# google-research/hyperbo

Hardware: AMD Instinct MI355X
Metric: GP NLL+grad evals/sec at N=8192 D=16 fp64 (higher is better)
Workload: dtype f64

## Files before the change

hyperbo_amd/csrc/chol.hip:

```cpp
#include "hbo_internal.h"
#include <type_traits>
#include <limits.h>
#include <string.h>

namespace {

#include "panel_dev.h"
#ifdef HBO_POTF2_TIMING
__device__ unsigned long long hbo_dbg_stamps[64];
__device__ unsigned long long hbo_dbg_wall[3 * 256];
__device__ unsigned long long hbo_dbg_trsm[3 * 128];
__device__ int hbo_dbg_trsm_panel = 36;
#define STAMP(i) do { if (threadIdx.x == 0) hbo_dbg_stamps[i] = __builtin_readcyclecounter(); } while (0)
#else
#define STAMP(i) do {} while (0)
#endif
#ifndef HBO_POTF2_WAVES
#define HBO_POTF2_WAVES 8
#endif
constexpr int POTF2_WAVES = HBO_POTF2_WAVES;
constexpr int POTF2_THREADS = 64 * POTF2_WAVES;
template <typename T>
__device__ __forceinline__ void potf2_body(const TaskDesc& t, int p, int* info_slot, unsigned char* smem) {
  typedef typename Mma<T>::acc_t acc_t;
  T* sT = reinterpret_cast<T*>(smem);
  T* sM = sT + 36 * TILE_ELEMS;
  T* sDinv = sM + TILE_ELEMS;
  const int64_t ld = t.ld;
  T* Ab = static_cast<T*>(t.A) + (int64_t)p * NB * ld + (int64_t)p * NB;
  T* Wb = static_cast<T*>(t.W) + (int64_t)p * NB * ld + (int64_t)p * NB;
  const int tid = threadIdx.x, lane = tid & 63, wave = tid >> 6;
  const int l15 = lane & 15, lq = lane >> 4;
  const int ei = (tid & 255) >> 4, ej = tid & 15;
  STAMP(0);
#ifdef HBO_POTF2_TIMING
  if (tid == 0 && blockIdx.x == 0 && p < 256) {
    hbo_dbg_wall[3 * p] = wall_clock64();
    hbo_dbg_wall[3 * p + 2] = ((unsigned long long)__builtin_amdgcn_s_getreg((20 << 0) | (0 << 6) | (31 << 11)) << 32) |
                              (unsigned)__builtin_amdgcn_s_getreg((4 << 0) | (0 << 6) | (31 << 11));
  }
#endif

  auto factor_leaf = [&](int jb, const acc_t* from_regs = nullptr) {
    T* dt = sT + tri_index(jb, jb) * TILE_ELEMS;
    acc_t acc;
    if (from_regs) acc = *from_regs;
    else {
#pragma unroll
      for (int r = 0; r < 4; ++r) acc[r] = dt[Mma<T>::crow(lane, r) * TS + l15];
    }
    const int bad = leaf_cholesky4<T>(acc, dt, sM, sDinv + jb * 16, Wb + (int64_t)(jb * 16) * ld + jb * 16, ld, lane);
    if (bad >= 0 && lane == 0) atomicMin(info_slot, p * NB + jb * 16 + bad + 1);
  };
  auto solve_tile = [&](int jb, int R) {
    T* xt = sT + tri_index(R, jb) * TILE_ELEMS;
    acc_t acc = {0, 0, 0, 0};
#pragma unroll
    for (int kk = 0; kk < 4; ++kk) acc = Mma<T>::mma(xt[l15 * TS + kk * 4 + lq], sM[l15 * TS + kk * 4 + lq], acc);
#pragma unroll
    for (int r = 0; r < 4; ++r) xt[Mma<T>::crow(lane, r) * TS + l15] = acc[r];
  };
  auto update_tile = [&](int jb, int I, int J) {
    T* ct = sT + tri_index(I, J) * TILE_ELEMS;
    const T* at = sT + tri_index(I, jb) * TILE_ELEMS;
    const T* bt = sT + tri_index(J, jb) * TILE_ELEMS;
    acc_t acc;
#pragma unroll
    for (int r = 0; r < 4; ++r) acc[r] = ct[Mma<T>::crow(lane, r) * TS + l15];
#pragma unroll
    for (int kk = 0; kk < 4; ++kk) acc = Mma<T>::mma(-at[l15 * TS + kk * 4 + lq], bt[l15 * TS + kk * 4 + lq], acc);
#pragma unroll
    for (int r = 0; r < 4; ++r) ct[Mma<T>::crow(lane, r) * TS + l15] = acc[r];
  };

  auto update_tile2 = [&](int jb, int I0, int J0, int I1, int J1) {
    T* c0 = sT + tri_index(I0, J0) * TILE_ELEMS;
    T* c1 = sT + tri_index(I1, J1) * TILE_ELEMS;
    const T* a0 = sT + tri_index(I0, jb) * TILE_ELEMS;
    const T* b0 = sT + tri_index(J0, jb) * TILE_ELEMS;
    const T* a1 = sT + tri_index(I1, jb) * TILE_ELEMS;
    const T* b1 = sT + tri_index(J1, jb) * TILE_ELEMS;
    acc_t x0, x1;
    T fa0[4], fb0[4], fa1[4], fb1[4];
#pragma unroll
    for (int r = 0; r < 4; ++r) { x0[r] = c0[Mma<T>::crow(lane, r) * TS + l15]; x1[r] = c1[Mma<T>::crow(lane, r) * TS + l15]; }
#pragma unroll
    for (int kk = 0; kk < 4; ++kk) {
      fa0[kk] = -a0[l15 * TS + kk * 4 + lq]; fb0[kk] = b0[l15 * TS + kk * 4 + lq];
      fa1[kk] = -a1[l15 * TS + kk * 4 + lq]; fb1[kk] = b1[l15 * TS + kk * 4 + lq];
    }
#pragma unroll
    for (int kk = 0; kk < 4; ++kk) { x0 = Mma<T>::mma(fa0[kk], fb0[kk], x0); x1 = Mma<T>::mma(fa1[kk], fb1[kk], x1); }
#pragma unroll
    for (int r = 0; r < 4; ++r) { c0[Mma<T>::crow(lane, r) * TS + l15] = x0[r]; c1[Mma<T>::crow(lane, r) * TS + l15] = x1[r]; }
  };

  int nleaf = 8;
  {
    const int64_t rows = (int64_t)t.n - (int64_t)p * NB;
    if (rows < NB) nleaf = rows <= 0 ? 0 : (int)((rows + 15) / 16);
    for (int jb = nleaf + wave; jb < 8; jb += POTF2_WAVES)
#pragma unroll
      for (int r = 0; r < 4; ++r) {
        const int row = Mma<T>::crow(lane, r);
        gst(Wb + (int64_t)(jb * 16 + row) * ld + jb * 16 + l15, row == l15 ? (T)1 : (T)0);
      }
    if (tid < NB && tid >= nleaf * 16) sDinv[tid] = (T)1;
  }
  const bool lead_tile0 = nleaf > 0;
  acc_t tile0 = {0, 0, 0, 0};
  if (wave == 0 && lead_tile0) {
#pragma unroll
    for (int r = 0; r < 4; ++r) {
      const int row = Mma<T>::crow(lane, r);
      const int rr = row > l15 ? row : l15, cc = row > l15 ? l15 : row;
      tile0[r] = gld(Ab + (int64_t)rr * ld + cc);
    }
  }
  constexpr int NSH = POTF2_THREADS / 256;
  const int sh = __builtin_amdgcn_readfirstlane(tid >> 8);
  T vload[36 / NSH];
  auto load_issue = [&](auto share) {
    constexpr int SH = decltype(share)::value;
    int tile = 0;
#pragma unroll
    for (int I = 0; I < 8; ++I)
#pragma unroll
      for (int J = 0; J <= I; ++J, ++tile) {
        if (tile % NSH != SH) continue;
        if (tile == 0 && lead_tile0) { vload[0] = (T)0; continue; }
        int r = ei, c = ej;
        if (I == J && ej > ei) { r = ej; c = ei; }
        vload[tile / NSH] = gld(Ab + (int64_t)(I * 16 + r) * ld + J * 16 + c);
      }
  };
  auto load_commit = [&](auto share) {
    constexpr int SH = decltype(share)::value;
#pragma unroll
    for (int k = 0; k < 36 / NSH; ++k)
      if (!(k == 0 && SH == 0 && lead_tile0)) sT[(k * NSH + SH) * TILE_ELEMS + ei * TS + ej] = vload[k];
  };
  static_assert(NSH == 1 || NSH == 2, "one or two 256-thread groups");
  if (NSH == 1 || sh == 0) load_issue(std::integral_constant<int, 0>());
  else load_issue(std::integral_constant<int, NSH - 1>());
  if (wave == 0 && lead_tile0) factor_leaf(0, &tile0);
  if (NSH == 1 || sh == 0) load_commit(std::integral_constant<int, 0>());
  else load_commit(std::integral_constant<int, NSH - 1>());
  STAMP(1);
  __syncthreads();
  STAMP(2);
  for (int jb = 0; jb < nleaf; ++jb) {
    for (int R = jb + 1 + wave; R < nleaf; R += POTF2_WAVES) solve_tile(jb, R);
    __syncthreads();
    STAMP(3 + 3 * jb);
    if (jb == nleaf - 1) break;
    {
      const int m = nleaf - 1 - jb;
      const int ntiles = m * (m + 1) / 2;
      constexpr int NH = POTF2_WAVES == 8 ? 6 : POTF2_WAVES - 1;
      const int hw = POTF2_WAVES == 8 ? (wave < 4 ? wave : wave - 1) : wave;
      const int n0 = (ntiles - 1 > 4 * NH + 1) ? (ntiles - 1 - (4 * NH + 1)) / POTF2_WAVES : 0;
      const int nshared = ntiles - n0;
      auto tile_of = [&](int tix, int& I, int& J) {
        int ii = 0;
        while ((ii + 1) * (ii + 2) / 2 <= tix) ++ii;
        I = jb + 1 + ii; J = jb + 1 + tix - ii * (ii + 1) / 2;
      };
      if (wave == 0) {
        update_tile(jb, jb + 1, jb + 1);
        factor_leaf(jb + 1);
        STAMP(4 + 3 * jb);
        for (int tix = nshared; tix < ntiles; ++tix) { int I, J; tile_of(tix, I, J); update_tile(jb, I, J); }
      } else if (!(POTF2_WAVES == 8 && wave == 4)) {
        int tix = hw;
        for (; tix + NH < nshared; tix += 2 * NH) {
          int I0, J0, I1, J1;
          tile_of(tix, I0, J0); tile_of(tix + NH, I1, J1);
          update_tile2(jb, I0, J0, I1, J1);
        }
        if (tix < nshared) { int I, J; tile_of(tix, I, J); update_tile(jb, I, J); }
      }
    }
    __syncthreads();
    STAMP(5 + 3 * jb);
  }
  STAMP(30);

  auto store_share = [&](auto share) {
    constexpr int SH = decltype(share)::value;
    int tile = 0;
#pragma unroll
    for (int I = 0; I < 8; ++I)
#pragma unroll
      for (int J = 0; J <= I; ++J, ++tile) {
        if (tile % NSH != SH) continue;
        T v = sT[tile * TILE_ELEMS + ei * TS + ej];
        if (I == J && ej > ei) v = (T)0;
        gst(Ab + (int64_t)(I * 16 + ei) * ld + J * 16 + ej, v);
      }
  };
  if (NSH == 1 || sh == 0) store_share(std::integral_constant<int, 0>());
  else store_share(std::integral_constant<int, NSH - 1>());
  STAMP(31);
  STAMP(32);
#ifdef HBO_POTF2_TIMING
  if (tid == 0 && blockIdx.x == 0 && p < 256) hbo_dbg_wall[3 * p + 1] = wall_clock64();
#endif
}
template <typename T>
__global__ __launch_bounds__(POTF2_THREADS) void potf2_kernel(const TaskDesc* tasks, int p, int* info, int* yield_flag, unsigned long long* tl) {
  extern __shared__ __attribute__((aligned(16))) unsigned char smem[];
  __builtin_amdgcn_s_setprio(3);
  const TaskDesc& t = tasks[blockIdx.x];
  if (p >= t.nblk) return;
  tl_begin(tl);
  int tok = 0;
  if (yield_flag && threadIdx.x == 0) tok = yield_enter(yield_flag);
  potf2_body<T>(t, p, info + blockIdx.x, smem);
  if (yield_flag) {
    __syncthreads();
    if (threadIdx.x == 0) yield_leave(yield_flag, tok);
  }
  tl_end(tl);
}

template <typename T>
constexpr int trsm_tile() { return sizeof(T) == 8 ? 256 : TILE_ELEMS; }
template <typename T>
__device__ __forceinline__ int trsm_at(int r, int c) { return sizeof(T) == 8 ? r * 16 + (c ^ ((r >> 1) << 1)) : r * TS + c; }
template <typename T>
constexpr int trsm_lds_bytes() { return (28 + 8 + 4) * trsm_tile<T>() * (int)sizeof(T); }
__device__ __forceinline__ int strict_index(int I, int J) { return I * (I - 1) / 2 + J; }

template <typename T, bool IDENT>
__device__ __forceinline__ void trsm_body(const TaskDesc& t, int p, int64_t row0, unsigned char* smem, bool stage) {
  typedef typename Mma<T>::acc_t acc_t;
  constexpr int TE = trsm_tile<T>();
  T* sLt = reinterpret_cast<T*>(smem);
  T* sWi = sLt + 28 * TE;
  T* sSc = sWi + 8 * TE;
  const int64_t ld = t.ld;
  const int tid = threadIdx.x, lane = tid & 63, wave = tid >> 6;
  const int l15 = lane & 15, lq = lane >> 4;
  const T* Lb = static_cast<const T*>(t.A) + (int64_t)p * NB * ld + (int64_t)p * NB;
  const T* Wb = static_cast<const T*>(t.W) + (int64_t)p * NB * ld + (int64_t)p * NB;

  const int64_t wrow0 = row0 + wave * 16;
  const int rg = IDENT ? (int)((wrow0 - (int64_t)p * NB) >> 4) : 0;
  T* Ap = IDENT ? nullptr : static_cast<T*>(t.A) + wrow0 * ld + (int64_t)p * NB;
  T* Wout = IDENT ? static_cast<T*>(t.W) + (int64_t)p * NB * ld + (int64_t)p * NB : nullptr;

  acc_t areg[8];
#pragma unroll
  for (int jb = 0; jb < 8; ++jb)
#pragma unroll
    for (int r = 0; r < 4; ++r) {
      const int row = Mma<T>::crow(lane, r);
      if (IDENT) areg[jb][r] = (rg == jb && row == l15) ? (T)1 : (T)0;
      else areg[jb][r] = gld(Ap + (int64_t)row * ld + jb * 16 + l15);
    }
  if (stage) {
    const int i = tid >> 4, j = tid & 15;
    int tile = 0;
#pragma unroll
    for (int I = 1; I < 8; ++I)
#pragma unroll
      for (int J = 0; J < I; ++J, ++tile)
        sLt[tile * TE + trsm_at<T>(i, j)] = gld(Lb + (int64_t)(I * 16 + i) * ld + J * 16 + j);
#pragma unroll
    for (int b = 0; b < 8; ++b)
      sWi[b * TE + trsm_at<T>(i, j)] = gld(Wb + (int64_t)(b * 16 + i) * ld + b * 16 + j);
  }
  if (stage) __syncthreads();

  T* sc = sSc + wave * TE;
  T xneg[8][4];
#pragma unroll
  for (int jb = 0; jb < 8; ++jb) {
    acc_t acc = areg[jb];
    acc_t acc2 = (acc_t){0, 0, 0, 0};
#pragma unroll
    for (int kb = 0; kb < 8; ++kb) {
      if (kb < jb) {
        const T* lt = sLt + strict_index(jb, kb) * TE;
#pragma unroll
        for (int kk = 0; kk < 4; ++kk) {
          const T bfrag = lt[trsm_at<T>(l15, kk * 4 + lq)];
          if (kb & 1) acc2 = Mma<T>::mma(xneg[kb][kk], bfrag, acc2);
          else acc = Mma<T>::mma(xneg[kb][kk], bfrag, acc);
        }
      }
    }
#pragma unroll
    for (int r = 0; r < 4; ++r) acc[r] += acc2[r];
    __builtin_amdgcn_wave_barrier();
#pragma unroll
    for (int r = 0; r < 4; ++r) sc[trsm_at<T>(Mma<T>::crow(lane, r), l15)] = acc[r];
    __builtin_amdgcn_wave_barrier();
    T ta[4];
#pragma unroll
    for (int kk = 0; kk < 4; ++kk) ta[kk] = sc[trsm_at<T>(l15, kk * 4 + lq)];
    acc_t x = (acc_t){0, 0, 0, 0};
    const T* wt = sWi + jb * TE;
#pragma unroll
    for (int kk = 0; kk < 4; ++kk) {
      const T bfrag = wt[trsm_at<T>(l15, kk * 4 + lq)];
      x = Mma<T>::mma(ta[kk], bfrag, x);
    }
#pragma unroll
    for (int r = 0; r < 4; ++r) {
      const int row = Mma<T>::crow(lane, r);
      if (IDENT) {
        if (rg != jb) gst(Wout + (int64_t)(jb * 16 + l15) * ld + rg * 16 + row, x[r]);
      } else {
        gst(Ap + (int64_t)row * ld + jb * 16 + l15, x[r]);
      }
    }
    if (jb < 7) {
      __builtin_amdgcn_wave_barrier();
#pragma unroll
      for (int r = 0; r < 4; ++r) sc[trsm_at<T>(Mma<T>::crow(lane, r), l15)] = x[r];
      __builtin_amdgcn_wave_barrier();
#pragma unroll
      for (int kk = 0; kk < 4; ++kk) xneg[jb][kk] = -sc[trsm_at<T>(l15, kk * 4 + lq)];
    }
  }
}
template <typename T, bool IDENT>
__global__ __launch_bounds__(256) void trsm_kernel(const TaskDesc* tasks, int p_arg, int* yield_tab, unsigned long long* tl) {
  extern __shared__ __attribute__((aligned(16))) unsigned char smem[];
  __builtin_amdgcn_s_setprio(3);
  const TaskDesc& t = tasks[blockIdx.z];
  const int p = IDENT ? p_arg + (int)blockIdx.y : p_arg;
  if (p >= t.nblk) return;
#ifdef HBO_POTF2_TIMING
  const bool dbg = !IDENT && p == hbo_dbg_trsm_panel && blockIdx.x < 128 && threadIdx.x == 0;
  if (dbg) {
    hbo_dbg_trsm[3 * blockIdx.x] = wall_clock64();
    hbo_dbg_trsm[3 * blockIdx.x + 2] = ((unsigned long long)__builtin_amdgcn_s_getreg((20 << 0) | (0 << 6) | (31 << 11)) << 32) |
                                       (unsigned)__builtin_amdgcn_s_getreg((4 << 0) | (0 << 6) | (31 << 11));
  }
#endif
  int64_t row0;
  if (IDENT) {
    row0 = (int64_t)p * NB + (int64_t)blockIdx.x * 64;
  } else {
    const int64_t first = (int64_t)(p + 1) * NB;
    const int64_t nrows = (int64_t)(t.nblk + 1) * NB - first;
    const int64_t bx = ((int64_t)blockIdx.x + 3 * (int64_t)blockIdx.z) % gridDim.x;
    if (bx * 64 >= nrows) return;
    row0 = first + bx * 64;
  }
  int tok = 0;
  tl_begin(tl);
  if (yield_tab && threadIdx.x == 0) tok = yield_enter(yield_tab);
  trsm_body<T, IDENT>(t, p, row0, smem, true);
  if (yield_tab) {
    __syncthreads();
    if (threadIdx.x == 0) yield_leave(yield_tab, tok);
  }
  tl_end(tl);
#ifdef HBO_POTF2_TIMING
  if (dbg) hbo_dbg_trsm[3 * blockIdx.x + 1] = wall_clock64();
#endif
}

template <typename T>
void set_attrs() {
  static unsigned long long seen = 0;
  if (!hbo_first_use_on_device(seen)) return;
  hipFuncSetAttribute(reinterpret_cast<const void*>(&potf2_kernel<T>),
                      hipFuncAttributeMaxDynamicSharedMemorySize, potf2_lds_bytes<T>());
  hipFuncSetAttribute(reinterpret_cast<const void*>(&trsm_kernel<T, false>),
                      hipFuncAttributeMaxDynamicSharedMemorySize, trsm_lds_bytes<T>());
  hipFuncSetAttribute(reinterpret_cast<const void*>(&trsm_kernel<T, true>),
                      hipFuncAttributeMaxDynamicSharedMemorySize, trsm_lds_bytes<T>());
}

template <typename T>
void potf2_t(const TaskDesc* tasks, int ntasks, int p, int* info, hipStream_t st, int* yield_flag, unsigned long long* tl) {
  set_attrs<T>();
  hipLaunchKernelGGL((potf2_kernel<T>), dim3(ntasks), dim3(POTF2_THREADS), potf2_lds_bytes<T>(), st, tasks, p, info,
                     yield_flag, tl);
}
template <typename T>
void trsm_t(const TaskDesc* tasks, int ntasks, int p, int max_nblk, hipStream_t st, int* yield_tab, unsigned long long* tl) {
  set_attrs<T>();
  const int nrows = (max_nblk + 1 - (p + 1)) * NB;
  if (nrows <= 0) return;
  hipLaunchKernelGGL((trsm_kernel<T, false>), dim3(nrows / 64, 1, ntasks), dim3(256), trsm_lds_bytes<T>(), st,
                     tasks, p, yield_tab, tl);
}
template <typename T>
void trtri_diag_t(const TaskDesc* tasks, int ntasks, int p_lo, int p_hi, hipStream_t st) {
  set_attrs<T>();
  if (p_hi <= p_lo) return;
  hipLaunchKernelGGL((trsm_kernel<T, true>), dim3(2, p_hi - p_lo, ntasks), dim3(256), trsm_lds_bytes<T>(), st,
                     tasks, p_lo, (int*)nullptr, (unsigned long long*)nullptr);
}

}

#ifdef HBO_POTF2_TIMING
void dbg_read_stamps(unsigned long long* host) { hipMemcpyFromSymbol(host, HIP_SYMBOL(hbo_dbg_stamps), sizeof(unsigned long long) * 64); }
extern "C" void hbo_dbg_trsm_wall(unsigned long long* host, int panel) {
  if (host) hipMemcpyFromSymbol(host, HIP_SYMBOL(hbo_dbg_trsm), sizeof(unsigned long long) * 3 * 128);
  else hipMemcpyToSymbol(HIP_SYMBOL(hbo_dbg_trsm_panel), &panel, sizeof(int));
}
extern "C" void hbo_dbg_potf2_wall(unsigned long long* host) { hipMemcpyFromSymbol(host, HIP_SYMBOL(hbo_dbg_wall), sizeof(unsigned long long) * 3 * 256); }
#endif
void launch_potf2(int dtype, const TaskDesc* tasks, int ntasks, int p, int* info, hipStream_t st, int* yield_flag, unsigned long long* tl) {
  if (dtype == HBO_F64) potf2_t<double>(tasks, ntasks, p, info, st, yield_flag, tl);
  else potf2_t<float>(tasks, ntasks, p, info, st, yield_flag, tl);
}
void launch_trsm(int dtype, const TaskDesc* tasks, int ntasks, int p, int max_nblk, hipStream_t st, int* yield_tab, unsigned long long* tl) {
  if (dtype == HBO_F64) trsm_t<double>(tasks, ntasks, p, max_nblk, st, yield_tab, tl);
  else trsm_t<float>(tasks, ntasks, p, max_nblk, st, yield_tab, tl);
}
void launch_trtri_diag(int dtype, const TaskDesc* tasks, int ntasks, int p_lo, int p_hi, hipStream_t st) {
  if (dtype == HBO_F64) trtri_diag_t<double>(tasks, ntasks, p_lo, p_hi, st);
  else trtri_diag_t<float>(tasks, ntasks, p_lo, p_hi, st);
}
```

Before: 93.93.

## Stream TRSM panel tiles through double-buffered LDS ring to raise occupancy

The fp64 panel triangular solve used to stage all 28 strict-lower L tiles plus 8 diagonal inverse tiles in LDS up front, about 80 KB per workgroup. It now keeps a two-slot ring holding one block-row of L tiles plus its diagonal inverse. The next row is prefetched into registers while the current row is processed, then committed after a workgroup barrier. This cuts LDS to about 40 KB so four workgroups can share a CU, and overlaps global loads with MMA work. The cost is a __syncthreads per block-row and more live registers for the prefetch buffer.

```diff
diff --git a/hyperbo_amd/csrc/chol.hip b/hyperbo_amd/csrc/chol.hip
--- a/hyperbo_amd/csrc/chol.hip
+++ b/hyperbo_amd/csrc/chol.hip
@@ -228,17 +228,18 @@
 constexpr int trsm_tile() { return sizeof(T) == 8 ? 256 : TILE_ELEMS; }
 template <typename T>
 __device__ __forceinline__ int trsm_at(int r, int c) { return sizeof(T) == 8 ? r * 16 + (c ^ ((r >> 1) << 1)) : r * TS + c; }
-template <typename T>
-constexpr int trsm_lds_bytes() { return (28 + 8 + 4) * trsm_tile<T>() * (int)sizeof(T); }
-__device__ __forceinline__ int strict_index(int I, int J) { return I * (I - 1) / 2 + J; }
+constexpr int TRSM_RING_TILES = 8;
+constexpr int TRSM_PIN_TILES = 4;
+template <typename T>
+constexpr int trsm_lds_bytes() { return (2 * TRSM_RING_TILES + 4) * trsm_tile<T>() * (int)sizeof(T); }
+static_assert(trsm_lds_bytes<double>() <= 40960, "fp64 panel solve: four workgroups per CU need <= 40 KB of LDS each");
 
 template <typename T, bool IDENT>
-__device__ __forceinline__ void trsm_body(const TaskDesc& t, int p, int64_t row0, unsigned char* smem, bool stage) {
+__device__ __forceinline__ void trsm_body(const TaskDesc& t, int p, int64_t row0, unsigned char* smem) {
   typedef typename Mma<T>::acc_t acc_t;
   constexpr int TE = trsm_tile<T>();
-  T* sLt = reinterpret_cast<T*>(smem);
-  T* sWi = sLt + 28 * TE;
-  T* sSc = sWi + 8 * TE;
+  T* sRing = reinterpret_cast<T*>(smem);
+  T* sSc = sRing + 2 * TRSM_RING_TILES * TE;
   const int64_t ld = t.ld;
   const int tid = threadIdx.x, lane = tid & 63, wave = tid >> 6;
   const int l15 = lane & 15, lq = lane >> 4;
@@ -259,30 +260,47 @@
       if (IDENT) areg[jb][r] = (rg == jb && row == l15) ? (T)1 : (T)0;
       else areg[jb][r] = gld(Ap + (int64_t)row * ld + jb * 16 + l15);
     }
-  if (stage) {
-    const int i = tid >> 4, j = tid & 15;
-    int tile = 0;
-#pragma unroll
-    for (int I = 1; I < 8; ++I)
-#pragma unroll
-      for (int J = 0; J < I; ++J, ++tile)
-        sLt[tile * TE + trsm_at<T>(i, j)] = gld(Lb + (int64_t)(I * 16 + i) * ld + J * 16 + j);
-#pragma unroll
-    for (int b = 0; b < 8; ++b)
-      sWi[b * TE + trsm_at<T>(i, j)] = gld(Wb + (int64_t)(b * 16 + i) * ld + b * 16 + j);
-  }
-  if (stage) __syncthreads();
+  const int sat = trsm_at<T>(tid >> 4, tid & 15);
+  const T* Ls = Lb + (int64_t)(tid >> 4) * ld + (tid & 15);
+  const T* Ws = Wb + (int64_t)(tid >> 4) * ld + (tid & 15);
+  auto row_load = [&](int I, T (&v)[TRSM_RING_TILES], int J0, int J1) {
+#pragma unroll
+    for (int J = 0; J < TRSM_RING_TILES - 1; ++J)
+      if (J >= J0 && J < J1 && J < I) v[J] = gld(Ls + (int64_t)(I * 16) * ld + J * 16);
+    if (J0 <= I && I < J1) v[TRSM_RING_TILES - 1] = gld(Ws + (int64_t)(I * 16) * ld + I * 16);
+  };
+  auto row_commit = [&](int I, const T (&v)[TRSM_RING_TILES]) {
+    T* buf = sRing + (I & 1) * TRSM_RING_TILES * TE;
+#pragma unroll
+    for (int J = 0; J < TRSM_RING_TILES - 1; ++J)
+      if (J < I) buf[J * TE + sat] = v[J];
+    buf[(TRSM_RING_TILES - 1) * TE + sat] = v[TRSM_RING_TILES - 1];
+  };
+  {
+    T v0[TRSM_RING_TILES], v1[TRSM_RING_TILES];
+    row_load(0, v0, 0, 8); row_load(1, v1, 0, 8);
+    row_commit(0, v0); row_commit(1, v1);
+  }
+  __syncthreads();
 
   T* sc = sSc + wave * TE;
   T xneg[8][4];
 #pragma unroll
   for (int jb = 0; jb < 8; ++jb) {
+    const T* ring = sRing + (jb & 1) * TRSM_RING_TILES * TE;
+    T nxt[TRSM_RING_TILES];
+    const bool ahead = jb >= 1 && jb < 7;
+    if (ahead) {
+      row_load(jb + 1, nxt, 0, TRSM_PIN_TILES);
+      __builtin_amdgcn_sched_barrier(0);
+      row_load(jb + 1, nxt, TRSM_PIN_TILES, 8);
+    }
     acc_t acc = areg[jb];
     acc_t acc2 = (acc_t){0, 0, 0, 0};
 #pragma unroll
     for (int kb = 0; kb < 8; ++kb) {
       if (kb < jb) {
-        const T* lt = sLt + strict_index(jb, kb) * TE;
+        const T* lt = ring + kb * TE;
 #pragma unroll
         for (int kk = 0; kk < 4; ++kk) {
           const T bfrag = lt[trsm_at<T>(l15, kk * 4 + lq)];
@@ -301,7 +319,7 @@
 #pragma unroll
     for (int kk = 0; kk < 4; ++kk) ta[kk] = sc[trsm_at<T>(l15, kk * 4 + lq)];
     acc_t x = (acc_t){0, 0, 0, 0};
-    const T* wt = sWi + jb * TE;
+    const T* wt = ring + (TRSM_RING_TILES - 1) * TE;
 #pragma unroll
     for (int kk = 0; kk < 4; ++kk) {
       const T bfrag = wt[trsm_at<T>(l15, kk * 4 + lq)];
@@ -323,6 +341,8 @@
       __builtin_amdgcn_wave_barrier();
 #pragma unroll
       for (int kk = 0; kk < 4; ++kk) xneg[jb][kk] = -sc[trsm_at<T>(l15, kk * 4 + lq)];
+      if (ahead) row_commit(jb + 1, nxt);
+      __syncthreads();
     }
   }
 }
@@ -354,7 +374,7 @@
   int tok = 0;
   tl_begin(tl);
   if (yield_tab && threadIdx.x == 0) tok = yield_enter(yield_tab);
-  trsm_body<T, IDENT>(t, p, row0, smem, true);
+  trsm_body<T, IDENT>(t, p, row0, smem);
   if (yield_tab) {
     __syncthreads();
     if (threadIdx.x == 0) yield_leave(yield_tab, tok);
```

Result: no change. 93.55 (-0.4%).
